# SandeepaInduwaraSamaranayake/SwinVox

Hardware: AMD Instinct MI355X
Metric: views/sec fwd+bwd SwinVox-T 224^2, 32^3 voxel, n_views=8 (higher is better)
Workload: dtype bf16; 1 GPU; SwinVox-T full pipeline (ResNet50[:layer3] || Swin multi-stage, cross-view attention, decoder, merger, refiner), fwd+2xBCE+bwd, train mode, B=64 samples x V=8 views of 224x224 per GPU; global_batch=64, n_views=8, images_per_gpu=512, parallelism=single GPU, launch=eager (one host launch per kernel, three streams)

## Files before the change

include/swinvox_hip.h:

```cpp
#ifndef SWINVOX_HIP_H
#define SWINVOX_HIP_H
#include <stddef.h>
#include <stdint.h>

#ifdef __cplusplus
extern "C" {
#endif

#define SV_OK 0
#define SV_ERR_INVALID (-1)
#define SV_ERR_LAUNCH (-2)

enum { SV_ACT_NONE = 0, SV_ACT_RELU = 1, SV_ACT_GELU = 2, SV_ACT_LRELU = 3 };
#define SV_BN_SLOTS 16
enum { SV_MATH_F32 = 0, SV_MATH_BF16 = 1, SV_MATH_FP8 = 2, SV_MATH_FP8_FULL = 3 };
enum { SV_F32 = 0, SV_BF16 = 1 };

const char* sv_last_error(void);
int sv_version(void);

typedef struct sv_geom {
  int N;
  int Di, Hi, Wi;
  int Do, Ho, Wo;
// ... 14 lines not shown
  double* stats;
  int act;
  float slope;
  const void* act_grad_src;
  int act_grad_kind;
  int ldc;
  int col_off;
} sv_epilogue;

int sv_conv_gather(const void* in, const void* w_packed, void* out, const sv_geom* g, const sv_epilogue* e,
                   int math, int act_dtype, void* stream);
int sv_set_conv_halo(int mode);
int sv_conv_halo_mode(void);
int sv_set_conv_halo_wgrad(int mode);
long long sv_conv_halo_launches(void);
enum { SV_PATH_GATHER = 0,
       SV_PATH_DENSE = 1,
       SV_PATH_WIDE = 2,
       SV_PATH_WIDE_GENERAL = 3,
       SV_PATH_HALO0 = 4, SV_PATH_HALO1 = 5, SV_PATH_HALO2 = 6,
       SV_PATH_HALO_BLOCKED_8X32 = 7, SV_PATH_HALO_BLOCKED_16X16 = 8,
       SV_PATH_WGRAD_TILED = 9,
       SV_PATH_WGRAD_WIDE = 10, SV_PATH_WGRAD_WIDE_SWAP = 11,
       SV_PATH_WGRAD_HALO = 12 };
enum { SV_OPERANDS_F32 = 0, SV_OPERANDS_BF16_F32 = 1, SV_OPERANDS_BF16 = 2 };
typedef struct sv_launch_plan {
  int path;
  int tile_rows, tile_cols;
  int operands;
  int vec;
  int grid_x, grid_y, block;
} sv_launch_plan;
int sv_conv_gather_plan(const void* in, const void* w, void* out, const sv_geom* g, const sv_epilogue* e, int math, int act_dtype, int transposed,
                        sv_launch_plan* plan);
int sv_conv_gather_is_wide(const void* in, const void* w, void* out, const sv_geom* g, const sv_epilogue* e, int math, int act_dtype);
int sv_tconv_gather(const void* in, const void* w_packed, void* out, const sv_geom* g, const sv_epilogue* e,
                    int math, int act_dtype, void* stream);
int sv_conv_wgrad_plan(const void* anchor, int lda, const void* gathered, const sv_geom* g, int cg_valid, int math, int act_dtype,
                       sv_launch_plan* plan);
int sv_conv_wgrad_is_wide(const void* anchor, int lda, const void* gathered, const sv_geom* g, int cg_valid, int math, int act_dtype);
size_t sv_conv_wgrad_workspace_floats(const sv_geom* g);
int sv_conv_wgrad(const void* anchor, int lda, const void* gathered, float* dw, const sv_geom* g, int cg_valid,
                  float* workspace, float* dbias , int math, int act_dtype,
                  void* stream);
int sv_quant_rows_e4m3(const void* src, int src_dtype, int rows, int K, int ld, void* dst_q, int Kp, float* scales, void* stream);
int sv_linear_fp8(const void* xq, const float* sx, const void* wq, const float* sw, void* out, int M, int K, int N, const sv_epilogue* e,
                  int act_dtype, void* stream);
// ... 233 lines not shown
```

swinvox_amd/csrc/igemm.hip:

```cpp
#include "common.h"
#include "conv_halo.h"
#include <stdlib.h>
#include <atomic>
#include <mutex>

namespace sv {

constexpr int PAD_F32 = 4;
#ifndef SV_PAD_BF16
#define SV_PAD_BF16 8
#endif
constexpr int PAD_BF16 = SV_PAD_BF16;

struct Geom {
  int N, Di, Hi, Wi, Do, Ho, Wo, Ci, Co, kd, kh, kw, sd, sh, sw, pd, ph, pw, ldi;
};
struct Epi {
  const float* bias; const void* residual; int ldr; const float* row_scale; int rows_per_scale;
  void* pre_act; double* stats; int act; float slope; const void* act_grad_src; int act_grad_kind; int ldc; int col_off;
};
struct ClassInfo {
  int o0[3];
  int cnt[3];
  int ib0[3];
// ... 545 lines not shown
    for (int mt = 0; mt < MT; ++mt)
#pragma unroll
      for (int nt = 0; nt < NT; ++nt) acc[mt][nt] = (f32x4){0.f, 0.f, 0.f, 0.f};
    for (int kt = 0; kt < nk; ++kt) {
      const int cur = kt & 1;
      if (kt + 1 < nk) load_slab(row0, col0, (kt + 1) * BK);
      mma_slab<true, MT, NT>(As + cur * STAGE, Bs + cur * STAGE, wm * MT * 16, wn * NT * 16, lane, acc);
      if (kt + 1 < nk) store_slab(cur ^ 1);
      __syncthreads();
    }
    int row0n = 0, col0n = 0;
    const bool more = tile_of(++it, row0n, col0n);
    if (more) load_slab(row0n, col0n, 0);
#ifdef SV_IG_PROBE_NOEPI
    if (acc[0][0][0] == 12345.678f) static_cast<AT*>(p.y)[0] = (AT)acc[0][0][1];
#else
    tile_epilogue<true, false, TL, AT>(p, ci, g.Do, g.Ho, g.Wo, Cs, red, acc, row0, col0, Mrows);
    __syncthreads();
#endif
    have = more; row0 = row0n; col0 = col0n;
  }
}

constexpr int GW_BN = 128, GW_BK = 64;
constexpr unsigned GW_NODRAW = 0xFFFFFFFFu;
typedef __attribute__((address_space(1))) const void* gw_gptr_t;
typedef __attribute__((address_space(3))) void* gw_lptr_t;

template <bool GENERAL, int WM, int NPROD, int NST>
__global__ __launch_bounds__((2 * WM + NPROD) * 64, 3) void gemm_wide_kernel(const IGemmArgs p, int ntiles, int* __restrict__ ctr) {
  constexpr int GW_NCONS = 2 * WM, GW_BM = 64 * WM, GW_A_BYTES = GW_BM * GW_BK * 2, GW_STAGE_BYTES = (GW_BM + GW_BN) * GW_BK * 2, GW_STAGES = NST;
  constexpr int PA = GW_BM / 8 / NPROD, PB = GW_BN / 8 / NPROD, LEAD = NST - 1;
  static_assert(PA % 2 == 0 && PB % 2 == 0 && (NST == 2 || NST == 3), "piece parity / ring depth");
  __shared__ __attribute__((aligned(1024))) char smem[GW_STAGES * GW_STAGE_BYTES + 64 + GW_NCONS * 1024];
  const __bf16* __restrict__ X = static_cast<const __bf16*>(p.x);
  const __bf16* __restrict__ Wt = static_cast<const __bf16*>(p.w);
  __bf16* __restrict__ Y = static_cast<__bf16*>(p.y);
  const Geom& g = p.g;
  const Epi& e = p.e;
  const int tid = threadIdx.x, lane = tid & 63, wave = tid >> 6;
  const int Mrows = g.N * g.Do * g.Ho * g.Wo, K = g.Ci, nk = K / GW_BK;
  const int tiles_n = (g.Co + GW_BN - 1) / GW_BN;
  const int xcd = blockIdx.x & 7, cq = ntiles >> 3, cr = ntiles & 7;
  const int cbase = xcd * cq + (xcd < cr ? xcd : cr), csize = cq + (xcd < cr ? 1 : 0);
  typedef __attribute__((address_space(3))) int lds_int;
  lds_int* mbox = (lds_int*)(smem + GW_STAGES * GW_STAGE_BYTES);
// ... 595 lines not shown
  if (g.Hi != g.Ho || g.Wi != g.Wo || g.ldi != g.Ci) return HaloPlan{};
  if (e.bias || e.residual || e.row_scale || e.pre_act || e.act != SV_ACT_NONE || e.act_grad_src || e.ldc != g.Co || e.col_off != 0) return HaloPlan{};
  if (dgrad && e.stats) return HaloPlan{};
  const bool k3 = g.kh == 3 && g.kw == 3 && g.ph == 1 && g.pw == 1, k4 = g.kh == 4 && g.kw == 4 && g.ph == 2 && g.pw == 2;
  if (dgrad && k4 && g.Ci == 64 && g.Co == 16) return conv_halo_plan(2, g.N, g.Hi, g.Wi);
  if (g.Co & 63) return HaloPlan{};
  if (k3) return g.Ci == 64 && g.Co == 64 ? conv_halo_plan(0, g.N, g.Hi, g.Wi) : conv_halo_blocked_plan(g.N, g.Hi, g.Wi, g.Ci, g.Co);
  if (!dgrad && k4 && g.Ci == 16 && g.Co == 64) return conv_halo_plan(1, g.N, g.Hi, g.Wi);
  return HaloPlan{};
}

static bool gemm_wide_ok(const IGemmArgs& a, long long M) {
  static const int enabled = [] { const char* v = getenv("SV_GEMM_WIDE"); return v ? atoi(v) : 1; }();
  const Epi& e = a.e;
  const int K = a.g.Ci, Co = a.g.Co;
  if (!enabled || K % GW_BK || K < 3 * GW_BK || Co < 128 || a.Ktot % 8) return false;
  if (enabled == 1 && e.stats && K < 1024) return false;
  if (enabled == 1 && e.act_grad_src && K < 384) return false;
  if (!rows_16_byte_aligned(a) || ((uintptr_t)a.w & 15)) return false;
  if ((e.stats && (e.residual || e.act_grad_src)) || (e.residual && e.act_grad_src)) return false;
  return (long long)cdiv(M, 256) * cdiv(Co, GW_BN) >= 256;
}

static GatherPlan plan_gather(const IGemmArgs& a, long long M, int ncls, int math, int act, bool tconv, bool counters) {
  const Geom& g = a.g;
  const int Co = g.Co;
  GatherPlan p{};
  const bool v8 = act == SV_BF16 && (g.Ci % 8) == 0 && (g.ldi % 8) == 0 && ((uintptr_t)a.x & 15) == 0;
  p.q.operands = math != SV_MATH_BF16 ? SV_OPERANDS_F32 : act != SV_BF16 ? SV_OPERANDS_BF16_F32 : SV_OPERANDS_BF16;
  p.q.vec = v8 ? 8 : 4;
  p.q.grid_y = 1;
  if (counters && (p.halo = plan_halo(a, math, act, tconv)).kind >= 0) {
    p.q.path = p.halo.kind < 3 ? SV_PATH_HALO0 + p.halo.kind : p.halo.th == 16 ? SV_PATH_HALO_BLOCKED_16X16 : SV_PATH_HALO_BLOCKED_8X32;
    p.q.tile_rows = p.halo.th; p.q.tile_cols = p.halo.tw; p.q.grid_x = p.halo.grid; p.q.block = 256;
    p.counters = true;
    return p;
  }
  const bool dense = !tconv && v8 && g.kd * g.kh * g.kw == 1 && g.sd == 1 && g.sh == 1 && g.sw == 1 &&
                     g.pd == 0 && g.ph == 0 && g.pw == 0 && g.Di == g.Do && g.Hi == g.Ho && g.Wi == g.Wo;
  if (dense && counters && gemm_wide_ok(a, M)) {
    p.q.path = a.e.residual || a.e.act_grad_src ? SV_PATH_WIDE_GENERAL : SV_PATH_WIDE;
    p.q.tile_rows = 256; p.q.tile_cols = GW_BN; p.q.grid_x = 256; p.q.block = 768;
    p.ntiles = cdiv(M, 256) * cdiv(Co, GW_BN);
    p.counters = true;
    return p;
  }
  bool use96 = false;
  if (Co % 96 == 0 && !a.e.stats) {
    auto est = [&](int bm, int bn) {
      const long long tn = cdiv(Co, bn), tiles = (long long)cdiv(M, bm) * tn * ncls;
      return (double)((tiles + 255) / 256) * bm * bn * (1.0 + 0.02 * (tn - 1));
    };
    const double e96 = est(128, 96), e64 = est(128, 64), e128 = Co > 64 ? est(128, 128) : 1e300;
    use96 = e96 <= e64 && e96 <= e128;
  }
  p.tile = Co <= 16 ? TILE_NARROW : use96 ? TILE_96 : Co > 64 && (long long)cdiv(M, 128) * cdiv(Co, 128) * ncls >= 384 ? TILE_BIG : TILE_DEFAULT;
  with_tile(p.tile, [&](auto tl) {
    typedef decltype(tl) TL;
    const int ntiles = cdiv(M, TL::BM) * cdiv(Co, TL::BN), resident = 256 * (TL::NTHR >= 512 ? 2 : 4);
    p.q.tile_rows = TL::BM; p.q.tile_cols = TL::BN; p.q.block = TL::NTHR;
    if (dense && Co > 16) { p.q.path = SV_PATH_DENSE; p.ntiles = ntiles; p.q.grid_x = resident < ntiles ? resident : ntiles; }
    else { p.q.path = SV_PATH_GATHER; p.q.grid_x = ntiles; p.q.grid_y = ncls; }
  });
  return p;
}

template <bool TCONV>
static void launch_gather(const GatherPlan& p, const IGemmArgs& a, int* ctr, hipStream_t s) {
  const dim3 grid(p.q.grid_x, p.q.grid_y), block(p.q.block);
  switch (p.q.path) {
    case SV_PATH_HALO0: case SV_PATH_HALO1: case SV_PATH_HALO2:
      conv_halo_launch(HaloConvArgs{a.x, a.w, a.y, a.e.stats, a.g.N, a.g.Hi, a.g.Wi, TCONV ? 1 : 0}, p.halo, ctr, s);
      return;
    case SV_PATH_HALO_BLOCKED_8X32: case SV_PATH_HALO_BLOCKED_16X16:
      conv_halo_blocked_launch(a.x, a.w, a.y, a.e.stats, a.g.N, a.g.Hi, a.g.Wi, a.g.Ci, a.g.Co, TCONV ? 1 : 0, p.halo, ctr, s);
      return;
    case SV_PATH_WIDE: hipLaunchKernelGGL((gemm_wide_kernel<false, 4, 4, 3>), grid, block, 0, s, a, p.ntiles, ctr); return;
    case SV_PATH_WIDE_GENERAL: hipLaunchKernelGGL((gemm_wide_kernel<true, 4, 4, 3>), grid, block, 0, s, a, p.ntiles, ctr); return;
    default: break;
  }
  with_tile(p.tile, [&](auto tl) {
    typedef decltype(tl) TL;
    if constexpr (!TCONV && TL::BN > 16) {
      if (p.q.path == SV_PATH_DENSE) { hipLaunchKernelGGL((gemm_dense_kernel<TL, __bf16, __bf16, 8>), grid, block, 0, s, a, p.ntiles); return; }
    }
    if (p.q.operands == SV_OPERANDS_F32) hipLaunchKernelGGL((igemm_kernel<false, TCONV, TL, float, float, 4>), grid, block, 0, s, a);
    else if (p.q.operands == SV_OPERANDS_BF16_F32) hipLaunchKernelGGL((igemm_kernel<true, TCONV, TL, float, float, 4>), grid, block, 0, s, a);
    else if (p.q.vec == 8) hipLaunchKernelGGL((igemm_kernel<true, TCONV, TL, __bf16, __bf16, 8>), grid, block, 0, s, a);
    else hipLaunchKernelGGL((igemm_kernel<true, TCONV, TL, __bf16, __bf16, 4>), grid, block, 0, s, a);
  });
}

static int gather_entry(const void* in, const void* w, void* out, const sv_geom* g, const sv_epilogue* e, int math, int act_dtype, bool transposed,
                        hipStream_t s, sv_launch_plan* query) {
  if (int rc = check_common(g, e, in, w, out, act_dtype)) return rc;
  SV_REQUIRE_ACT(act_dtype);
  SV_REQUIRE(act_dtype == SV_F32 || math == SV_MATH_BF16, "igemm: bf16 activations require SV_MATH_BF16");
  IGemmArgs a{};
  a.x = in; a.w = w; a.y = out; a.g = to_geom(g); a.e = to_epi(e);
  a.Ktot = g->kd * g->kh * g->kw * g->Ci;
  long long M = (long long)g->N * g->Do * g->Ho * g->Wo;
// ... 8 lines not shown
          const int r[3] = {rd, rh, rw};
          ClassInfo c{};
          long long m = g->N;
          for (int ax = 0; ax < 3; ++ax) {
            c.r[ax] = r[ax];
            c.T[ax] = r[ax] < Kx[ax] ? (Kx[ax] - r[ax] + S[ax] - 1) / S[ax] : 0;
            int o0 = ((r[ax] - P[ax]) % S[ax] + S[ax]) % S[ax];
            c.o0[ax] = o0;
            c.cnt[ax] = o0 < O[ax] ? (O[ax] - o0 + S[ax] - 1) / S[ax] : 0;
            c.ib0[ax] = (o0 + P[ax] - r[ax]) / S[ax];
            m *= c.cnt[ax];
          }
          if (m > M) M = m;
          a.cls[ncls++] = c;
        }
  }
  GatherPlan p = plan_gather(a, M, ncls, math, act_dtype, transposed, true);
  if (query) { *query = p.q; return SV_OK; }
  if (M == 0) return SV_OK;
  int* ctr = p.counters ? gemm_wide_counters() : nullptr;
  if (p.counters && !ctr) p = plan_gather(a, M, ncls, math, act_dtype, transposed, false);
  if (transposed) launch_gather<true>(p, a, ctr, s);
  else launch_gather<false>(p, a, ctr, s);
  if (p.q.path >= SV_PATH_HALO0) return check_launch(transposed ? "sv_tconv_gather (halo tiles)" : "sv_conv_gather (halo tiles)");
  return check_launch(transposed ? "sv_tconv_gather" : "sv_conv_gather");
}

struct WGradWideArgs {
  const __bf16* P; int ldp; int pcols; const __bf16* Q; int ldq; int qcols;
  float* dw; int ld_dw;
  float* dbias;
  int nslices, ntiles, tiles_p, groups;
};

constexpr int GW_NCONS = 8, GW_NPROD = 4, GW_NTHR = (GW_NCONS + GW_NPROD) * 64, GW_STAGES = 3;
constexpr int GW_A_BYTES = 256 * GW_BK * 2, GW_STAGE_BYTES = (256 + GW_BN) * GW_BK * 2;
template <bool SWAP>
__global__ __launch_bounds__(GW_NTHR, 3) void wgrad_wide_kernel(const WGradWideArgs p) {
  __shared__ __attribute__((aligned(1024))) char smem[GW_STAGES * GW_STAGE_BYTES];
  const int tid = threadIdx.x, lane = tid & 63, wave = tid >> 6;
  const int bl = xcd_remap(blockIdx.x, gridDim.x);
  const int tile = bl % p.ntiles, grp = bl / p.ntiles;
  const int p0 = (tile % p.tiles_p) * 256, q0 = (tile / p.tiles_p) * 128;
  const int sbase = p.nslices / p.groups, srem = p.nslices % p.groups;
  const int s0 = grp * sbase + (grp < srem ? grp : srem), nsl = sbase + (grp < srem ? 1 : 0);
  if (nsl <= 0) return;

// ... 244 lines not shown
    int blocks = cdiv(total, 256); if (blocks > 2048) blocks = 2048;
    hipLaunchKernelGGL(wgrad_unpack_kernel, dim3(blocks), dim3(256), 0, s, workspace, dw, g->Co, g->Ci, cg_valid, taps);
  }
  return check_launch(p.q.path == SV_PATH_WGRAD_HALO ? "sv_conv_wgrad (halo tiles)" : "sv_conv_wgrad");
}

}

using namespace sv;

extern "C" int sv_conv_gather(const void* in, const void* w, void* out, const sv_geom* g, const sv_epilogue* e,
                              int math, int act_dtype, void* stream) {
  return gather_entry(in, w, out, g, e, math, act_dtype, false, (hipStream_t)stream, nullptr);
}
extern "C" int sv_tconv_gather(const void* in, const void* w, void* out, const sv_geom* g, const sv_epilogue* e,
                               int math, int act_dtype, void* stream) {
  return gather_entry(in, w, out, g, e, math, act_dtype, true, (hipStream_t)stream, nullptr);
}
extern "C" int sv_conv_gather_plan(const void* in, const void* w, void* out, const sv_geom* g, const sv_epilogue* e, int math, int act_dtype,
                                   int transposed, sv_launch_plan* plan) {
  SV_REQUIRE(plan, "conv_gather_plan: null plan");
  return gather_entry(in, w, out, g, e, math, act_dtype, transposed != 0, nullptr, plan);
}
extern "C" int sv_conv_gather_is_wide(const void* in, const void* w, void* out, const sv_geom* g, const sv_epilogue* e, int math, int act_dtype) {
  sv_launch_plan q;
  return sv_conv_gather_plan(in, w, out, g, e, math, act_dtype, 0, &q) == SV_OK && (q.path == SV_PATH_WIDE || q.path == SV_PATH_WIDE_GENERAL);
}

extern "C" size_t sv_conv_wgrad_workspace_floats(const sv_geom* g) {
  const int taps = g->kd * g->kh * g->kw;
  return taps == 1 ? 0 : (size_t)g->Co * taps * g->Ci;
}
extern "C" int sv_conv_wgrad(const void* anchor, int lda, const void* gathered, float* dw, const sv_geom* g, int cg_valid,
                             float* workspace, float* dbias, int math, int act_dtype, void* stream) {
  return wgrad_entry(anchor, lda, gathered, dw, g, cg_valid, workspace, dbias, math, act_dtype, (hipStream_t)stream, nullptr);
}
extern "C" int sv_conv_wgrad_plan(const void* anchor, int lda, const void* gathered, const sv_geom* g, int cg_valid, int math, int act_dtype,
                                  sv_launch_plan* plan) {
  SV_REQUIRE(plan, "conv_wgrad_plan: null plan");
  return wgrad_entry(anchor, lda, gathered, nullptr, g, cg_valid, nullptr, nullptr, math, act_dtype, nullptr, plan);
}
extern "C" int sv_conv_wgrad_is_wide(const void* anchor, int lda, const void* gathered, const sv_geom* g, int cg_valid, int math, int act_dtype) {
  sv_launch_plan q;
  return sv_conv_wgrad_plan(anchor, lda, gathered, g, cg_valid, math, act_dtype, &q) == SV_OK &&
         (q.path == SV_PATH_WGRAD_WIDE || q.path == SV_PATH_WGRAD_WIDE_SWAP);
}
// ... 41 lines not shown
```

swinvox_amd/csrc/stencil.hip:

```cpp
#include "common.h"
#include <map>
#include <mutex>
#include <type_traits>

namespace sv {

constexpr int TZ = 4, TY = 8, TX = 8;
constexpr int HZ = TZ + 2, HY = TY + 2, HX = TX + 2;
constexpr int HPOS = HZ * HY * HX;
constexpr int NVOX = TZ * TY * TX;
typedef __attribute__((address_space(3))) bf16x4 lds_bf16x4_t;

__device__ __forceinline__ bf16x4 to_bf16x4(float4 v) {
  bf16x4 b;
  b[0] = (__bf16)v.x; b[1] = (__bf16)v.y; b[2] = (__bf16)v.z; b[3] = (__bf16)v.w;
  return b;
}
__device__ __forceinline__ bf16x4 to_bf16x4(bf16x4 v) { return v; }

__device__ __forceinline__ int xcd_first_tile() {
  const int n = gridDim.x, b = blockIdx.x;
  return (n & 7) == 0 ? (b & 7) * (n >> 3) + (b >> 3) : b;
}

// ... 571 lines not shown
        const int tap = dz * 9 + p0 + pi;
#pragma unroll
        for (int gg = 0; gg < G; ++gg) {
          const f32x4 o = hand[((pi * 3 + dz) * G + gg) * 64];
          const int cm = gg * 16 + lr;
          const int grp = cm / p.c_stride, within = cm - grp * p.c_stride;
          const int ci = grp * p.c_valid + within;
          if (within < p.c_valid && ci < p.cin) {
#pragma unroll
            for (int j = 0; j < 4; ++j) {
              const int co = lg * 4 + j;
              if (co < p.cout) atomicAdd(dst + ((size_t)co * p.cin + ci) * 27 + tap, acc[pi][dz][gg][j] + o[j]);
            }
          }
        }
      }
    }
  }
}

struct TConv4Args {
  const __bf16* x; const __bf16* w;
  const float* bias; __bf16* out; double* stats; int cout; int I, D, H, W, nbricks;
};
constexpr int T4_JZ = 4, T4_JY = 4, T4_JX = 8, T4_HZ = 6, T4_HY = 6, T4_HX = 10, T4_HPOS = T4_HZ * T4_HY * T4_HX;

__global__ __launch_bounds__(256, 2) void tconv4s2_fwd_kernel(const TConv4Args p) {
  __shared__ __attribute__((aligned(16))) __bf16 Xs[T4_HPOS * 32];
  __shared__ __attribute__((aligned(16))) __bf16 Ws[8 * 8 * 256];
  __shared__ __attribute__((aligned(16))) __bf16 Os[8 * 8 * 16 * 8];
  __shared__ float red[4][16];
  const int tid = threadIdx.x, lane = tid & 63, wave = tid >> 6;
  const int lr = lane & 15, lg = lane >> 4;
  for (int i = tid; i < 8 * 8 * 256 / 8; i += 256) {
    const int c8 = (i & 3) * 8, t = (i >> 2) & 7, co = (i >> 5) & 7, cls = i >> 8;
    const int az = cls >> 2, ay = (cls >> 1) & 1, ax = cls & 1, dz = t >> 2, dy = (t >> 1) & 1, dx = t & 1;
    const int kz = az ? 2 - 2 * dz : 3 - 2 * dz, ky = ay ? 2 - 2 * dy : 3 - 2 * dy, kx = ax ? 2 - 2 * dx : 3 - 2 * dx;
    bf16x8 v = VecN<__bf16, 8>::zero();
    if (co < p.cout) v = *reinterpret_cast<const bf16x8*>(p.w + ((size_t)co * 64 + (kz * 4 + ky) * 4 + kx) * 32 + c8);
    *reinterpret_cast<bf16x8*>(Ws + ((cls * 8 + co) * 256) + t * 32 + c8) = v;
  }
  float bias4[4];
#pragma unroll
  for (int j = 0; j < 4; ++j) bias4[j] = (p.bias && lg < 2 && lg * 4 + j < p.cout) ? p.bias[lg * 4 + j] : 0.f;
  double st1[8], st2[8];
#pragma unroll
// ... 26 lines not shown
        if (lr < 8) b[tt] = *reinterpret_cast<const bf16x8*>(Ws + (cls * 8 + lr) * 256 + tt * 32 + lg * 8);
      }
#pragma unroll 2
      for (int g = 0; g < 8; ++g) {
        const int jz = g >> 1, jy = (g & 1) * 2 + yy;
        const int base = ((jz + az) * T4_HY + (jy + ay)) * T4_HX + (xx + ax);
        f32x4 acc = (f32x4){0.f, 0.f, 0.f, 0.f};
#pragma unroll
        for (int tt = 0; tt < 8; ++tt) {
          const int off = ((tt >> 2) * T4_HY + ((tt >> 1) & 1)) * T4_HX + (tt & 1);
          const bf16x8 a = *reinterpret_cast<const bf16x8*>(Xs + (base + off) * 32 + lg * 8);
          acc = __builtin_amdgcn_mfma_f32_16x16x32_bf16(b[tt], a, acc, 0, 0, 0);
        }
        if (lg < 2) {
          bf16x4 o;
#pragma unroll
          for (int j = 0; j < 4; ++j) o[j] = (__bf16)(acc[j] + bias4[j]);
          const int oz = 2 * jz + az, oy = 2 * jy + ay, ox = 2 * xx + ax;
          *reinterpret_cast<bf16x4*>(Os + ((oz * 8 + oy) * 16 + ox) * 8 + lg * 4) = o;
        }
      }
    }
    __syncthreads();
#pragma unroll
    for (int k = 0; k < 4; ++k) {
      const int v = tid + 256 * k;
      const int ox = v & 15, oy = (v >> 4) & 7, oz = v >> 7;
      const bf16x8 o = *reinterpret_cast<const bf16x8*>(Os + v * 8);
      const size_t pos = (((size_t)img * (2 * p.D) + 2 * z0 + oz) * (2 * p.H) + 2 * y0 + oy) * (2 * p.W) + 2 * x0 + ox;
      *reinterpret_cast<bf16x8*>(p.out + pos * 8) = o;
      if (p.stats) {
#pragma unroll
        for (int c = 0; c < 8; ++c) { const double f = (double)(float)o[c]; st1[c] += f; st2[c] += f * f; }
      }
    }
    __syncthreads();
  }
  if (p.stats) {
#pragma unroll
    for (int c = 0; c < 8; ++c) {
      float a = (float)st1[c], b2 = (float)st2[c];
      a = wave_sum(a); b2 = wave_sum(b2);
      if (lane == 0) { red[wave][c] = a; red[wave][8 + c] = b2; }
    }
    __syncthreads();
    if (tid < 16 && (tid & 7) < p.cout) {
      const float v = red[0][tid] + red[1][tid] + red[2][tid] + red[3][tid];
      double* st = p.stats + (size_t)(blockIdx.x % SV_BN_SLOTS) * 2 * p.cout;
      atomicAdd(st + (tid >> 3) * p.cout + (tid & 7), (double)v);
    }
  }
}

}

using namespace sv;

static int resident_per_cu(const void* kernel, int threads = 256) {
  static std::mutex mu;
  static std::map<const void*, int> cache;
  std::lock_guard<std::mutex> lk(mu);
  auto it = cache.find(kernel);
  if (it != cache.end()) return it->second;
  int n = 0;
  if (hipOccupancyMaxActiveBlocksPerMultiprocessor(&n, kernel, threads, 0) != hipSuccess || n < 1) { (void)hipGetLastError(); n = 1; }
  cache[kernel] = n;
  return n;
}

static int stencil_check(int I, int D, int H, int W) {
  SV_REQUIRE(I > 0 && D % 8 == 0 && H % TY == 0 && W % TX == 0, "stencil3: grid %dx%dx%d must be a multiple of the 8x8x8 brick", D, H, W);
  return SV_OK;
}

#define SV_STENCIL_LAUNCH(GG, NTT, VV)                                                                                     \
  do {                                                                                                                    \
    constexpr int nthr = StencilBrickF<GG>::NTHR;                                                                         \
    const int nt_ = I * (D / StencilBrickF<GG>::TZV) * (H / TY) * (W / TX);                                               \
    a.ntiles = nt_;                                                                                                       \
// ... 56 lines not shown
  const bool sweep = sweep_env ? atoi(sweep_env) != 0 : true;
  SV_DISPATCH_ACT(act_dtype,
    const void* k1 = sweep ? (const void*)stencil3_wgrad_sweep_kernel<1, AT> : (const void*)stencil3_wgrad_kernel<1, AT>;
    const void* k3 = sweep ? (const void*)stencil3_wgrad_sweep_kernel<3, AT> : (const void*)stencil3_wgrad_kernel<3, AT>;
    const int per_cu = groups == 1 ? resident_per_cu(k1, StencilBrick<1>::NTHR) : resident_per_cu(k3, StencilBrick<3>::NTHR);
    const int resident = 256 * per_cu;
    const int blocks = ntiles < resident ? ntiles : resident;
    StencilWArgsT<AT> a{static_cast<const AT*>(x), ldx, cin_load, x_plane_stride, static_cast<const AT*>(dy), lddy, cout_load, dw, workspace, dbias, cout, cin, c_stride, c_valid,
                        I, D, H, W, ntiles};
    if (groups == 1 && sweep) hipLaunchKernelGGL((stencil3_wgrad_sweep_kernel<1, AT>), dim3(blocks), dim3(StencilBrick<1>::NTHR), 0, s, a);
    else if (groups == 1) hipLaunchKernelGGL((stencil3_wgrad_kernel<1, AT>), dim3(blocks), dim3(StencilBrick<1>::NTHR), 0, s, a);
    else if (sweep) hipLaunchKernelGGL((stencil3_wgrad_sweep_kernel<3, AT>), dim3(blocks), dim3(StencilBrick<3>::NTHR), 0, s, a);
    else hipLaunchKernelGGL((stencil3_wgrad_kernel<3, AT>), dim3(blocks), dim3(StencilBrick<3>::NTHR), 0, s, a););
  if (workspace) hipLaunchKernelGGL(stencil_wgrad_fold_kernel, dim3(cdiv(cout * cin * 27, 256)), dim3(256), 0, s, workspace, dw, cout * cin * 27);
  return check_launch("sv_stencil3_wgrad");
}

extern "C" int sv_tconv4s2_fwd(const void* x, const void* w_packed, const float* bias, void* out, double* stats, int I, int D, int H, int W,
                               int cin, int cout, void* stream) {
  SV_REQUIRE(x && w_packed && out && I > 0, "tconv4s2_fwd: null argument");
  SV_REQUIRE(cin == 32 && cout > 0 && cout <= 8, "tconv4s2_fwd: built for 32 input and <= 8 output channels (got %d -> %d)", cin, cout);
  SV_REQUIRE(D % T4_JZ == 0 && H % T4_JY == 0 && W % T4_JX == 0, "tconv4s2_fwd: input grid %dx%dx%d must be a multiple of the 4x4x8 brick", D, H, W);
  SV_REQUIRE((((uintptr_t)x | (uintptr_t)w_packed | (uintptr_t)out) & 15) == 0, "tconv4s2_fwd: operands must be 16-byte aligned");
  TConv4Args a{static_cast<const __bf16*>(x), static_cast<const __bf16*>(w_packed), bias, static_cast<__bf16*>(out), stats, cout, I, D, H, W,
               I * (D / T4_JZ) * (H / T4_JY) * (W / T4_JX)};
  const int blocks = a.nbricks < 512 ? a.nbricks : 512;
  hipLaunchKernelGGL(tconv4s2_fwd_kernel, dim3(blocks), dim3(256), 0, (hipStream_t)stream, a);
  return check_launch("sv_tconv4s2_fwd");
}
```

swinvox_amd/hip.py:

```python
from __future__ import annotations

import ctypes as C
import os
import threading

import torch

_HERE = os.path.dirname(os.path.abspath(__file__))
LIB_PATH = os.environ.get("SV_HIP_LIB") or os.path.join(_HERE, "libswinvox_hip.so")

ACT_NONE, ACT_RELU, ACT_GELU, ACT_LRELU = 0, 1, 2, 3
MATH_F32, MATH_BF16, MATH_FP8, MATH_FP8_FULL = 0, 1, 2, 3
F32, BF16 = 0, 1


class Geom(C.Structure):
    _fields_ = [(n, C.c_int) for n in ("N", "Di", "Hi", "Wi", "Do", "Ho", "Wo", "Ci", "Co", "kd", "kh", "kw",
                                        "sd", "sh", "sw", "pd", "ph", "pw", "ldi")]


class Epilogue(C.Structure):
    _fields_ = [("bias", C.c_void_p), ("residual", C.c_void_p), ("ldr", C.c_int), ("row_scale", C.c_void_p),
                ("rows_per_scale", C.c_int), ("pre_act", C.c_void_p), ("stats", C.c_void_p), ("act", C.c_int),
                ("slope", C.c_float), ("act_grad_src", C.c_void_p), ("act_grad_kind", C.c_int), ("ldc", C.c_int),
                ("col_off", C.c_int)]


class LaunchPlan(C.Structure):
    _fields_ = [(n, C.c_int) for n in ("path", "tile_rows", "tile_cols", "operands", "vec", "grid_x", "grid_y", "block")]


(PATH_GATHER, PATH_DENSE, PATH_WIDE, PATH_WIDE_GENERAL, PATH_HALO0, PATH_HALO1, PATH_HALO2, PATH_HALO_BLOCKED_8X32, PATH_HALO_BLOCKED_16X16,
 PATH_WGRAD_TILED, PATH_WGRAD_WIDE, PATH_WGRAD_WIDE_SWAP, PATH_WGRAD_HALO) = range(13)
OPERANDS_F32, OPERANDS_BF16_F32, OPERANDS_BF16 = 0, 1, 2


class PackDesc(C.Structure):
    _fields_ = [("src", C.c_void_p), ("dst", C.c_void_p), ("A", C.c_int), ("B", C.c_int), ("T", C.c_int), ("swap", C.c_int),
                ("rows_out", C.c_int), ("inner_out", C.c_int), ("block0", C.c_int), ("reserved", C.c_int)]


class AugSample(C.Structure):
    _fields_ = [("bg", C.c_float * 3), ("jitter_value", C.c_float * 3), ("jitter_order", C.c_int * 3), ("noise", C.c_float * 3),
                ("perm", C.c_int * 3), ("mean", C.c_float * 3), ("std", C.c_float * 3)]


_P, _I, _L, _F, _U, _D = C.c_void_p, C.c_int, C.c_longlong, C.c_float, C.c_uint32, C.c_double
_ACT_TYPED = {
    "sv_conv_gather", "sv_tconv_gather", "sv_conv_wgrad", "sv_stencil3_fwd", "sv_stencil3_wgrad", "sv_colsum",
    "sv_layernorm_fwd", "sv_layernorm_quant_fwd", "sv_layernorm_quant_mx_fwd", "sv_layernorm_bwd", "sv_ln_image_fwd", "sv_ln_image_bwd", "sv_bn_stats", "sv_scale_shift_act", "sv_bn_bwd", "sv_scale_shift_act_signs", "sv_bn_bwd_signs", "sv_scale_shift_act2_signs", "sv_bn_bwd2_signs",
    "sv_window_attention_fwd", "sv_window_attention_fwd_mxq", "sv_window_attention_bwd", "sv_cross_view_attention_fwd", "sv_cross_view_attention_bwd",
    "sv_transpose", "sv_add_n", "sv_axpby", "sv_relu_bwd", "sv_maxpool2d_fwd", "sv_maxpool2d_bwd", "sv_avgpool2_fwd", "sv_avgpool2_bwd",
    "sv_decoder_seed_fwd", "sv_decoder_seed_bwd", "sv_maxpool3d_fwd", "sv_maxpool3d_bwd", "sv_dropout", "sv_rowscale",
    "sv_dwconv2x2_fwd", "sv_dwconv2x2_bwd", "sv_upsample3to7_add_fwd", "sv_upsample3to7_bwd",
    "sv_cva_downsample_fwd", "sv_cva_downsample_bwd", "sv_cva_upsample_add_fwd", "sv_cva_upsample_bwd", "sv_decoder_head_fwd", "sv_decoder_head_bwd",
    "sv_merge_views_fwd", "sv_merge_views_bwd", "sv_stem_space_to_depth", "sv_encoder_prep", "sv_encoder_prep_bwd", "sv_bn_act_maxpool_fwd", "sv_bn_maxpool_bwd", "sv_bn_act_maxpool3d_fwd", "sv_bn_maxpool3d_bwd", "sv_head_pack_x", "sv_head_unpack_dx", "sv_swin_attn_block_fwd", "sv_swin_attn_block_fwd_mx", "sv_swin_attn_block_bwd",
# ... 55 lines not shown
    "sv_bn_stats": (_I, [_P, _L, _I, _I, _P]),
    "sv_bn_finalize": (_I, [_P, _L, _P, _P, _P, _P, _F, _F, _I, _P, _P, _P, _P, _I]),
    "sv_scale_shift_act": (_I, [_P, _I, _P, _P, _P, _I, _P, _I, _L, _I, _I, _F]),
    "sv_bn_bwd": (_I, [_P, _I, _P, _I, _P, _I, _P, _P, _P, _L, _I, _I, _F, _I, _P, _I, _P, _I, _P, _P, _P, _P, _P]),
    "sv_bn_signs_supported": (_I, None, [_I]),
    "sv_scale_shift_act_signs": (_I, [_P, _I, _P, _P, _P, _I, _P, _I, _L, _I, _I, _F, _P]),
    "sv_bn_bwd_signs": (_I, [_P, _I, _P, _P, _I, _P, _P, _P, _L, _I, _I, _F, _I, _P, _I, _P, _I, _P, _P, _P]),
    "sv_scale_shift_act2_signs": (_I, [_P, _I, _P, _P, _P, _I, _P, _P, _P, _I, _L, _I, _P]),
    "sv_bn_bwd2_signs": (_I, [_P, _I, _P, _P, _I, _P, _P, _P, _P, _I, _P, _P, _P, _L, _I, _P, _I, _P, _I, _P, _P, _P, _P, _P, _P]),
    "sv_window_attention_fwd": (_I, [_P, _P, _P, _I, _I, _I, _I, _I, _I, _I]),
    "sv_window_attention_fwd_mxq": (_I, [_P, _P, _P, _I, _I, _I, _I, _I, _I, _I, _P, _I, _P]),
    "sv_window_attention_bwd_workspace_floats": (C.c_size_t, None, [_I]),
    "sv_window_attention_windows_per_group": (_I, None, [_I, _I, _I, _I, _I, _I]),
    "sv_window_attention_bwd": (_I, [_P, _P, _P, _P, _P, _P, _I, _I, _I, _I, _I, _I, _I]),
    "sv_stem_space_to_depth": (_I, [_P, _P, _I]),
    "sv_bn_act_maxpool_fwd": (_I, [_P, _P, _P, _P, _P, _I, _I, _I, _I, _I, _F]),
    "sv_bn_maxpool_bwd": (_I, [_P, _P, _P, _P, _P, _P, _P, _P, _I, _I, _I, _I, _I, _F, _I, _P, _P, _P, _P]),
    "sv_bn_act_maxpool3d_fwd": (_I, [_P, _P, _P, _P, _P, _I, _I, _I, _I, _I, _I, _F]),
    "sv_bn_maxpool3d_bwd": (_I, [_P, _P, _P, _P, _P, _P, _P, _P, _I, _I, _I, _I, _I, _I, _F, _I, _P, _P, _P, _P]),
    "sv_set_conv_halo": (_I, None, [_I]),
    "sv_conv_halo_mode": (_I, None),
    "sv_set_conv_halo_wgrad": (_I, None, [_I]),
    "sv_conv_halo_launches": (_L, None),
    "sv_encoder_prep": (_I, [_P, _I, _P, _P, _I, _I]),
    "sv_encoder_prep_bwd": (_I, [_P, _P, _P, _I, _I, _I]),
    "sv_head_pack_x": (_I, [_P, _P, _I, _I]),
    "sv_head_unpack_dx": (_I, [_P, _P, _I, _I]),
    "sv_stem_pack": (_I, [_P, _P, _I]),
    "sv_stem_unpack_grad": (_I, [_P, _P]),
    "sv_stem_native": (_I, [_P, _P]),
    "sv_merger_pack": (_I, [_P, _P, _I, _I, _I, _I]),
    "sv_swin_mlp_supported": (_I, None, [_I]),
    "sv_swin_mlp_pack": (_I, [_P, _P, _P, _I]),
    "sv_swin_mlp_fwd": (_I, [_P, _P, _P, _P, _P, _P, _P, _P, _I, _L, _I, _F]),
    "sv_swin_mlp_bwd": (_I, [_P, _P, _P, _P, _P, _P, _P, _P, _I, _P, _P, _L, _I, _F]),
    "sv_swin_mlp_wgrad": (_I, [_P, _P, _P, _P, _P, _P, _P, _P, _I, _P, _P, _P, _P, _L, _I, _F]),
    "sv_swin_mlp_mx_supported": (_I, None, [_I]),
    "sv_swin_mlp_mx_pack_bytes": (_L, None, [_I]),
    "sv_swin_mlp_mx_pack": (_I, [_P, _P, _P, _P, _P, _I]),
    "sv_swin_mlp_fwd_mx": (_I, [_P, _P, _P, _P, _P, _P, _P, _P, _I, _L, _I, _F]),
    "sv_swin_mlp_mx_launches": (_L, None),
    "sv_swin_mlp_bwd_mx_supported": (_I, None, [_I]),
    "sv_swin_mlp_bwd_mx_pack_bytes": (_L, None, [_I]),
    "sv_swin_mlp_bwd_mx_pack": (_I, [_P, _P, _P, _P, _P, _P, _P, _I]),
    "sv_swin_mlp_bwd_mx": (_I, [_P, _P, _P, _P, _P, _P, _P, _P, _I, _P, _P, _L, _I, _F]),
    "sv_swin_mlp_bwd_mx_launches": (_L, None),
# ... 191 lines not shown
```

Before: 4999 views/s.

## Route tiny-M dense GEMMs and 4x4x4 stride-2 tconv fwd/dgrad to specialized kernels

```diff
diff --git a/include/swinvox_hip.h b/include/swinvox_hip.h
--- a/include/swinvox_hip.h
+++ b/include/swinvox_hip.h
@@ -60,7 +60,11 @@
        SV_PATH_HALO_BLOCKED_8X32 = 7, SV_PATH_HALO_BLOCKED_16X16 = 8,
        SV_PATH_WGRAD_TILED = 9,
        SV_PATH_WGRAD_WIDE = 10, SV_PATH_WGRAD_WIDE_SWAP = 11,
-       SV_PATH_WGRAD_HALO = 12 };
+       SV_PATH_WGRAD_HALO = 12,
+       SV_PATH_SKINNY = 13,
+       SV_PATH_TCONV_BRICK = 14,
+       SV_PATH_TCONV_BRICK_DGRAD = 15 };
+int sv_set_tail_kernels(int mask);
 enum { SV_OPERANDS_F32 = 0, SV_OPERANDS_BF16_F32 = 1, SV_OPERANDS_BF16 = 2 };
 typedef struct sv_launch_plan {
   int path;
diff --git a/swinvox_amd/csrc/igemm.hip b/swinvox_amd/csrc/igemm.hip
--- a/swinvox_amd/csrc/igemm.hip
+++ b/swinvox_amd/csrc/igemm.hip
@@ -1,5 +1,6 @@
 #include "common.h"
 #include "conv_halo.h"
+#include "stencil.h"
 #include <stdlib.h>
 #include <atomic>
 #include <mutex>
@@ -591,6 +592,103 @@
   }
 }
 
+constexpr int SK_NW = 8, SK_NS = 4, SK_BN = 16, SK_BK = 64;
+template <int MB> struct SkinnyStage { bf16x8 w[2]; bf16x8 x[MB][2]; };
+
+template <int MB>
+__global__ __launch_bounds__(SK_NW * 64, 2) void gemm_skinny_kernel(const IGemmArgs p) {
+  __shared__ __attribute__((aligned(16))) float part[SK_NW][MB][64][4];
+  const Geom& g = p.g;
+  const Epi& e = p.e;
+  const int tid = threadIdx.x, lane = tid & 63, wave = tid >> 6, lr = lane & 15, lg = lane >> 4;
+  const int M = g.N * g.Do * g.Ho * g.Wo, nch = g.Ci / SK_BK;
+  const int n0 = blockIdx.x * SK_BN;
+  const __bf16* __restrict__ wrow = static_cast<const __bf16*>(p.w) + (size_t)(n0 + lr) * p.Ktot + lg * 8;
+  const __bf16* __restrict__ xrow[MB];
+  bool xok[MB];
+#pragma unroll
+  for (int mb = 0; mb < MB; ++mb) {
+    const int m = mb * 16 + lr;
+    xok[mb] = m < M;
+    xrow[mb] = static_cast<const __bf16*>(p.x) + (size_t)(xok[mb] ? m : 0) * g.ldi + lg * 8;
+  }
+  SkinnyStage<MB> st[SK_NS];
+  auto load = [&](SkinnyStage<MB>& s, int i) {
+    const int c = wave + SK_NW * i;
+    if (c < nch) {
+      const int k0 = c * SK_BK;
+#pragma unroll
+      for (int ks = 0; ks < 2; ++ks) s.w[ks] = VecN<__bf16, 8>::load(wrow + k0 + ks * 32);
+#pragma unroll
+      for (int mb = 0; mb < MB; ++mb)
+#pragma unroll
+        for (int ks = 0; ks < 2; ++ks) s.x[mb][ks] = xok[mb] ? VecN<__bf16, 8>::load(xrow[mb] + k0 + ks * 32) : VecN<__bf16, 8>::zero();
+    } else {
+#pragma unroll
+      for (int ks = 0; ks < 2; ++ks) {
+        s.w[ks] = VecN<__bf16, 8>::zero();
+#pragma unroll
+        for (int mb = 0; mb < MB; ++mb) s.x[mb][ks] = VecN<__bf16, 8>::zero();
+      }
+    }
+  };
+  f32x4 acc[MB];
+#pragma unroll
+  for (int mb = 0; mb < MB; ++mb) acc[mb] = (f32x4){0.f, 0.f, 0.f, 0.f};
+#pragma unroll
+  for (int s = 0; s < SK_NS; ++s) load(st[s], s);
+  const int nmine = wave < nch ? (nch - wave + SK_NW - 1) / SK_NW : 0;
+  for (int i0 = 0; i0 < nmine; i0 += SK_NS) {
+#pragma unroll
+    for (int s = 0; s < SK_NS; ++s) {
+#pragma unroll
+      for (int ks = 0; ks < 2; ++ks)
+#pragma unroll
+        for (int mb = 0; mb < MB; ++mb)
+          acc[mb] = __builtin_amdgcn_mfma_f32_16x16x32_bf16(st[s].w[ks], st[s].x[mb][ks], acc[mb], 0, 0, 0);
+      load(st[s], i0 + s + SK_NS);
+    }
+  }
+#pragma unroll
+  for (int mb = 0; mb < MB; ++mb) *reinterpret_cast<f32x4*>(&part[wave][mb][lane][0]) = acc[mb];
+  __syncthreads();
+  const int m = wave * 16 + lr;
+  if (wave >= MB || m >= M) return;
+  f32x4 sum = *reinterpret_cast<const f32x4*>(&part[0][wave][lane][0]);
+#pragma unroll
+  for (int w = 1; w < SK_NW; ++w) sum += *reinterpret_cast<const f32x4*>(&part[w][wave][lane][0]);
+  const int n = n0 + lg * 4;
+  const size_t o = (size_t)m * e.ldc + e.col_off + n;
+  float v[4];
+#pragma unroll
+  for (int j = 0; j < 4; ++j) v[j] = sum[j] + (e.bias ? e.bias[n + j] : 0.f);
+  if (e.act_grad_src) {
+    float a[4];
+    ldnf<4>(static_cast<const __bf16*>(e.act_grad_src) + o, a);
+    if (e.act_grad_kind == SV_ACT_GELU) {
+#pragma unroll
+      for (int j = 0; j < 4; j += 2) {
+        const f32x2 dg = gelu_grad_fast2((f32x2){a[j], a[j + 1]});
+        v[j] *= dg[0]; v[j + 1] *= dg[1];
+      }
+    } else {
+#pragma unroll
+      for (int j = 0; j < 4; ++j) v[j] *= act_grad_t<true>(a[j], e.act_grad_kind, e.slope);
+    }
+  }
+  if (e.act == SV_ACT_GELU) {
+#pragma unroll
+    for (int j = 0; j < 4; j += 2) {
+      const f32x2 gl = gelu_fast2((f32x2){v[j], v[j + 1]});
+      v[j] = gl[0]; v[j + 1] = gl[1];
+    }
+  } else {
+#pragma unroll
+    for (int j = 0; j < 4; ++j) v[j] = apply_act_t<true>(v[j], e.act, e.slope);
+  }
+  stnf<4>(static_cast<__bf16*>(p.y) + o, v);
+}
+
 constexpr int GW_BN = 128, GW_BK = 64;
 constexpr unsigned GW_NODRAW = 0xFFFFFFFFu;
 typedef __attribute__((address_space(1))) const void* gw_gptr_t;
@@ -1232,6 +1330,41 @@
   return (long long)cdiv(M, 256) * cdiv(Co, GW_BN) >= 256;
 }
 
+static std::atomic<int>& tail_mask() {
+  static std::atomic<int> m{[] { const char* v = getenv("SV_TAIL_KERNELS"); return v ? atoi(v) & 15 : 7; }()};
+  return m;
+}
+constexpr long long SK_MIN_KCO = 1LL << 16;
+static bool skinny_ok(const IGemmArgs& a, long long M) {
+  const int mask = tail_mask().load(std::memory_order_relaxed);
+  const Epi& e = a.e;
+  if (!(mask & 1) || M < 1 || M > 64 || a.g.Ci < SK_BK || a.g.Ci % SK_BK || a.g.Co % SK_BN) return false;
+  if (e.residual || e.row_scale || e.pre_act || e.stats) return false;
+  if (!rows_16_byte_aligned(a) || (((uintptr_t)a.w | (uintptr_t)a.x) & 15) || a.Ktot % 8) return false;
+  return (mask & 8) != 0 || (long long)a.g.Ci * a.g.Co >= SK_MIN_KCO;
+}
+static bool tconv_brick_ok(const IGemmArgs& a, int math, int act) {
+  const Geom& g = a.g;
+  const Epi& e = a.e;
+  if (!(tail_mask().load(std::memory_order_relaxed) & 4) || math != SV_MATH_BF16 || act != SV_BF16) return false;
+  if (g.kd != 4 || g.kh != 4 || g.kw != 4 || g.sd != 2 || g.sh != 2 || g.sw != 2 || g.pd != 1 || g.ph != 1 || g.pw != 1) return false;
+  if (g.Do != 2 * g.Di || g.Ho != 2 * g.Hi || g.Wo != 2 * g.Wi || g.Di % 4 || g.Hi % 4 || g.Wi % 8) return false;
+  if (g.Ci != 32 || g.ldi != 32 || g.Co > 8 || e.ldc != g.Co || e.col_off != 0) return false;
+  if (e.residual || e.row_scale || e.pre_act || e.stats || e.act != SV_ACT_NONE || e.act_grad_src) return false;
+  return (((uintptr_t)a.x | (uintptr_t)a.w | (uintptr_t)a.y) & 15) == 0;
+}
+
+static bool tconv_brick_dgrad_ok(const IGemmArgs& a, int math, int act) {
+  const Geom& g = a.g;
+  const Epi& e = a.e;
+  if (!(tail_mask().load(std::memory_order_relaxed) & 2) || math != SV_MATH_BF16 || act != SV_BF16) return false;
+  if (g.kd != 4 || g.kh != 4 || g.kw != 4 || g.sd != 2 || g.sh != 2 || g.sw != 2 || g.pd != 1 || g.ph != 1 || g.pw != 1) return false;
+  if (g.Di != 2 * g.Do || g.Hi != 2 * g.Ho || g.Wi != 2 * g.Wo || g.Do % 4 || g.Ho % 4 || g.Wo % 8) return false;
+  if (g.Ci != 8 || g.ldi != 8 || g.Co != 32 || e.ldc != 32 || e.col_off != 0) return false;
+  if (e.bias || e.residual || e.row_scale || e.pre_act || e.stats || e.act != SV_ACT_NONE || e.act_grad_src) return false;
+  return (((uintptr_t)a.x | (uintptr_t)a.w | (uintptr_t)a.y) & 15) == 0;
+}
+
 static GatherPlan plan_gather(const IGemmArgs& a, long long M, int ncls, int math, int act, bool tconv, bool counters) {
   const Geom& g = a.g;
   const int Co = g.Co;
@@ -1248,6 +1381,20 @@
   }
   const bool dense = !tconv && v8 && g.kd * g.kh * g.kw == 1 && g.sd == 1 && g.sh == 1 && g.sw == 1 &&
                      g.pd == 0 && g.ph == 0 && g.pw == 0 && g.Di == g.Do && g.Hi == g.Ho && g.Wi == g.Wo;
+  if (tconv && tconv_brick_ok(a, math, act)) {
+    const int nbricks = g.N * (g.Di / 4) * (g.Hi / 4) * (g.Wi / 8);
+    p.q.path = SV_PATH_TCONV_BRICK; p.q.tile_rows = 4 * 4 * 8; p.q.tile_cols = 8; p.q.grid_x = nbricks < 512 ? nbricks : 512; p.q.block = 256;
+    return p;
+  }
+  if (!tconv && tconv_brick_dgrad_ok(a, math, act)) {
+    const int nbricks = g.N * (g.Do / 4) * (g.Ho / 4) * (g.Wo / 8);
+    p.q.path = SV_PATH_TCONV_BRICK_DGRAD; p.q.tile_rows = 4 * 4 * 8; p.q.tile_cols = 32; p.q.grid_x = nbricks < 512 ? nbricks : 512; p.q.block = 256;
+    return p;
+  }
+  if (dense && math == SV_MATH_BF16 && skinny_ok(a, M)) {
+    p.q.path = SV_PATH_SKINNY; p.q.tile_rows = 64; p.q.tile_cols = SK_BN; p.q.grid_x = Co / SK_BN; p.q.block = SK_NW * 64;
+    return p;
+  }
   if (dense && counters && gemm_wide_ok(a, M)) {
     p.q.path = a.e.residual || a.e.act_grad_src ? SV_PATH_WIDE_GENERAL : SV_PATH_WIDE;
     p.q.tile_rows = 256; p.q.tile_cols = GW_BN; p.q.grid_x = 256; p.q.block = 768;
@@ -1287,6 +1434,17 @@
       return;
     case SV_PATH_WIDE: hipLaunchKernelGGL((gemm_wide_kernel<false, 4, 4, 3>), grid, block, 0, s, a, p.ntiles, ctr); return;
     case SV_PATH_WIDE_GENERAL: hipLaunchKernelGGL((gemm_wide_kernel<true, 4, 4, 3>), grid, block, 0, s, a, p.ntiles, ctr); return;
+    case SV_PATH_SKINNY: {
+      const int M = a.g.N * a.g.Do * a.g.Ho * a.g.Wo;
+      if (M <= 16) hipLaunchKernelGGL(gemm_skinny_kernel<1>, grid, block, 0, s, a);
+      else if (M <= 32) hipLaunchKernelGGL(gemm_skinny_kernel<2>, grid, block, 0, s, a);
+      else hipLaunchKernelGGL(gemm_skinny_kernel<4>, grid, block, 0, s, a);
+      return;
+    }
+    case SV_PATH_TCONV_BRICK_DGRAD: tconv4s2_dgrad_launch(a.x, a.w, a.y, a.g.N, a.g.Do, a.g.Ho, a.g.Wo, p.q.grid_x, s); return;
+    case SV_PATH_TCONV_BRICK:
+      tconv4s2_fwd_launch(a.x, a.w, a.e.bias, a.y, nullptr, a.g.N, a.g.Di, a.g.Hi, a.g.Wi, a.g.Co, a.e.ldc, p.q.grid_x, s);
+      return;
     default: break;
   }
   with_tile(p.tile, [&](auto tl) {
@@ -1341,7 +1499,7 @@
   if (p.counters && !ctr) p = plan_gather(a, M, ncls, math, act_dtype, transposed, false);
   if (transposed) launch_gather<true>(p, a, ctr, s);
   else launch_gather<false>(p, a, ctr, s);
-  if (p.q.path >= SV_PATH_HALO0) return check_launch(transposed ? "sv_tconv_gather (halo tiles)" : "sv_conv_gather (halo tiles)");
+  if (p.q.path >= SV_PATH_HALO0 && p.q.path <= SV_PATH_HALO_BLOCKED_16X16) return check_launch(transposed ? "sv_tconv_gather (halo tiles)" : "sv_conv_gather (halo tiles)");
   return check_launch(transposed ? "sv_tconv_gather" : "sv_conv_gather");
 }
 
@@ -1632,6 +1790,11 @@
   SV_REQUIRE(plan, "conv_gather_plan: null plan");
   return gather_entry(in, w, out, g, e, math, act_dtype, transposed != 0, nullptr, plan);
 }
+extern "C" int sv_set_tail_kernels(int mask) {
+  SV_REQUIRE(mask >= 0 && mask <= 15, "sv_set_tail_kernels: mask %d (bit 0 skinny dense, bit 1 brick data gradient, bit 2 transposed-convolution brick, bit 3 skinny below its threshold)", mask);
+  sv::tail_mask().store(mask, std::memory_order_relaxed);
+  return SV_OK;
+}
 extern "C" int sv_conv_gather_is_wide(const void* in, const void* w, void* out, const sv_geom* g, const sv_epilogue* e, int math, int act_dtype) {
   sv_launch_plan q;
   return sv_conv_gather_plan(in, w, out, g, e, math, act_dtype, 0, &q) == SV_OK && (q.path == SV_PATH_WIDE || q.path == SV_PATH_WIDE_GENERAL);
diff --git a/swinvox_amd/csrc/stencil.h b/swinvox_amd/csrc/stencil.h
--- /dev/null
+++ b/swinvox_amd/csrc/stencil.h
@@ -0,0 +1,10 @@
+#pragma once
+#include <hip/hip_runtime.h>
+
+namespace sv {
+
+void tconv4s2_fwd_launch(const void* x, const void* w, const float* bias, void* out, double* stats, int I, int D, int H, int W, int cout, int ldc,
+                         int blocks, hipStream_t stream);
+void tconv4s2_dgrad_launch(const void* dy, const void* w, void* dx, int I, int D, int H, int W, int blocks, hipStream_t stream);
+
+}
diff --git a/swinvox_amd/csrc/stencil.hip b/swinvox_amd/csrc/stencil.hip
--- a/swinvox_amd/csrc/stencil.hip
+++ b/swinvox_amd/csrc/stencil.hip
@@ -1,4 +1,5 @@
 #include "common.h"
+#include "stencil.h"
 #include <map>
 #include <mutex>
 #include <type_traits>
@@ -617,6 +618,7 @@
 struct TConv4Args {
   const __bf16* x; const __bf16* w;
   const float* bias; __bf16* out; double* stats; int cout; int I, D, H, W, nbricks;
+  int ldc;
 };
 constexpr int T4_JZ = 4, T4_JY = 4, T4_JX = 8, T4_HZ = 6, T4_HY = 6, T4_HX = 10, T4_HPOS = T4_HZ * T4_HY * T4_HX;
 
@@ -689,6 +691,22 @@
       }
     }
     __syncthreads();
+    if (p.ldc != 8) {
+      const int pieces = 2 * p.cout;
+      for (int q = tid; q < 64 * pieces; q += 256) {
+        const int row = q / pieces, pc = q - row * pieces, oy = row & 7, oz = row >> 3;
+        bf16x8 o;
+#pragma unroll
+        for (int j = 0; j < 8; ++j) {
+          const int el = pc * 8 + j, ox = el / p.cout, c = el - ox * p.cout;
+          o[j] = Os[(row * 16 + ox) * 8 + c];
+        }
+        const size_t pos = (((size_t)img * (2 * p.D) + 2 * z0 + oz) * (2 * p.H) + 2 * y0 + oy) * (2 * p.W) + 2 * x0;
+        *reinterpret_cast<bf16x8*>(p.out + pos * p.cout + pc * 8) = o;
+      }
+      __syncthreads();
+      continue;
+    }
 #pragma unroll
     for (int k = 0; k < 4; ++k) {
       const int v = tid + 256 * k;
@@ -719,9 +737,100 @@
   }
 }
 
+struct TConv4DgradArgs {
+  const __bf16* dy; const __bf16* w;
+  __bf16* dx;
+  int I, D, H, W, nbricks;
+};
+constexpr int T4D_HZ = 10, T4D_HY = 10, T4D_HX = 18, T4D_SLOTS = T4D_HZ * T4D_HY * T4D_HX, T4D_ROW = 12, T4D_PLANE = T4D_HZ * T4D_HY * T4D_ROW;
+constexpr int T4D_PF = (T4D_SLOTS + 255) / 256;
+
+__global__ __launch_bounds__(256, 2) void tconv4s2_dgrad_kernel(const TConv4DgradArgs p) {
+  __shared__ __attribute__((aligned(16))) __bf16 Ys[2 * T4D_PLANE * 8];
+  const int tid = threadIdx.x, lane = tid & 63, wave = tid >> 6;
+  const int lr = lane & 15, lg = lane >> 4;
+  bf16x8 b[16][2];
+#pragma unroll
+  for (int ks = 0; ks < 16; ++ks)
+#pragma unroll
+    for (int ct = 0; ct < 2; ++ct)
+      b[ks][ct] = *reinterpret_cast<const bf16x8*>(p.w + ((size_t)((lr >> 2) * 8 + ct * 4 + (lr & 3)) * 64 + ks * 4 + lg) * 8);
+  const int bz = p.D / T4_JZ, by = p.H / T4_JY, bx = p.W / T4_JX;
+  const int Dy = 2 * p.D, Hy = 2 * p.H, Wy = 2 * p.W;
+  int img, z0, y0, x0;
+  auto decode = [&](int brick) {
+    int t = brick;
+    x0 = (t % bx) * T4_JX; t /= bx;
+    y0 = (t % by) * T4_JY; t /= by;
+    z0 = (t % bz) * T4_JZ; img = t / bz;
+  };
+  bf16x8 pf[T4D_PF];
+  auto fetch = [&](int brick) {
+    int fi, fz, fy, fx;
+    { int t = brick; fx = (t % bx) * T4_JX; t /= bx; fy = (t % by) * T4_JY; t /= by; fz = (t % bz) * T4_JZ; fi = t / bz; }
+#pragma unroll
+    for (int i = 0; i < T4D_PF; ++i) {
+      const int h = tid + 256 * i;
+      const int hx = h % T4D_HX, t2 = h / T4D_HX, hy = t2 % T4D_HY, hz = t2 / T4D_HY;
+      const int z = 2 * fz - 1 + hz, y = 2 * fy - 1 + hy, x = 2 * fx - 1 + hx;
+      pf[i] = VecN<__bf16, 8>::zero();
+      if (h < T4D_SLOTS && (unsigned)z < (unsigned)Dy && (unsigned)y < (unsigned)Hy && (unsigned)x < (unsigned)Wy)
+        pf[i] = *reinterpret_cast<const bf16x8*>(p.dy + ((((size_t)fi * Dy + z) * Hy + y) * Wy + x) * 8);
+    }
+  };
+  int brick = blockIdx.x;
+  if (brick < p.nbricks) fetch(brick);
+  const int yy = lr >> 3, xx = lr & 7;
+  const int lane_slot = (lg & 1) * T4D_PLANE + xx + (lg >> 1);
+  while (brick < p.nbricks) {
+#pragma unroll
+    for (int i = 0; i < T4D_PF; ++i) {
+      const int h = tid + 256 * i;
+      const int hx = h % T4D_HX, row = h / T4D_HX;
+      if (h < T4D_SLOTS) *reinterpret_cast<bf16x8*>(Ys + ((hx & 1) * T4D_PLANE + row * T4D_ROW + (hx >> 1)) * 8) = pf[i];
+    }
+    __syncthreads();
+    decode(brick);
+    const int next = brick + gridDim.x;
+    if (next < p.nbricks) fetch(next);
+#pragma unroll 1
+    for (int g = 0; g < 2; ++g) {
+      const int jy = 2 * g + yy;
+      f32x4 acc[2] = {(f32x4){0.f, 0.f, 0.f, 0.f}, (f32x4){0.f, 0.f, 0.f, 0.f}};
+#pragma unroll
+      for (int ks = 0; ks < 16; ++ks) {
+        const int row = (2 * wave + (ks >> 2)) * T4D_HY + 2 * jy + (ks & 3);
+        const bf16x8 a = *reinterpret_cast<const bf16x8*>(Ys + (row * T4D_ROW + lane_slot) * 8);
+#pragma unroll
+        for (int ct = 0; ct < 2; ++ct) acc[ct] = __builtin_amdgcn_mfma_f32_16x16x32_bf16(b[ks][ct], a, acc[ct], 0, 0, 0);
+      }
+      bf16x8 o;
+#pragma unroll
+      for (int j = 0; j < 4; ++j) { o[j] = (__bf16)acc[0][j]; o[4 + j] = (__bf16)acc[1][j]; }
+      const size_t pos = (((size_t)img * p.D + z0 + wave) * p.H + y0 + jy) * p.W + x0 + xx;
+      *reinterpret_cast<bf16x8*>(p.dx + pos * 32 + lg * 8) = o;
+    }
+    __syncthreads();
+    brick = next;
+  }
+}
+
 }
 
 using namespace sv;
+
+void sv::tconv4s2_dgrad_launch(const void* dy, const void* w, void* dx, int I, int D, int H, int W, int blocks, hipStream_t stream) {
+  TConv4DgradArgs a{static_cast<const __bf16*>(dy), static_cast<const __bf16*>(w), static_cast<__bf16*>(dx), I, D, H, W,
+                    I * (D / T4_JZ) * (H / T4_JY) * (W / T4_JX)};
+  hipLaunchKernelGGL(tconv4s2_dgrad_kernel, dim3(blocks), dim3(256), 0, stream, a);
+}
+
+void sv::tconv4s2_fwd_launch(const void* x, const void* w, const float* bias, void* out, double* stats, int I, int D, int H, int W, int cout, int ldc,
+                             int blocks, hipStream_t stream) {
+  TConv4Args a{static_cast<const __bf16*>(x), static_cast<const __bf16*>(w), bias, static_cast<__bf16*>(out), stats, cout, I, D, H, W,
+               I * (D / T4_JZ) * (H / T4_JY) * (W / T4_JX), ldc};
+  hipLaunchKernelGGL(tconv4s2_fwd_kernel, dim3(blocks), dim3(256), 0, stream, a);
+}
 
 static int resident_per_cu(const void* kernel, int threads = 256) {
   static std::mutex mu;
@@ -824,9 +933,7 @@
   SV_REQUIRE(cin == 32 && cout > 0 && cout <= 8, "tconv4s2_fwd: built for 32 input and <= 8 output channels (got %d -> %d)", cin, cout);
   SV_REQUIRE(D % T4_JZ == 0 && H % T4_JY == 0 && W % T4_JX == 0, "tconv4s2_fwd: input grid %dx%dx%d must be a multiple of the 4x4x8 brick", D, H, W);
   SV_REQUIRE((((uintptr_t)x | (uintptr_t)w_packed | (uintptr_t)out) & 15) == 0, "tconv4s2_fwd: operands must be 16-byte aligned");
-  TConv4Args a{static_cast<const __bf16*>(x), static_cast<const __bf16*>(w_packed), bias, static_cast<__bf16*>(out), stats, cout, I, D, H, W,
-               I * (D / T4_JZ) * (H / T4_JY) * (W / T4_JX)};
-  const int blocks = a.nbricks < 512 ? a.nbricks : 512;
-  hipLaunchKernelGGL(tconv4s2_fwd_kernel, dim3(blocks), dim3(256), 0, (hipStream_t)stream, a);
+  const int nbricks = I * (D / T4_JZ) * (H / T4_JY) * (W / T4_JX);
+  tconv4s2_fwd_launch(x, w_packed, bias, out, stats, I, D, H, W, cout, 8, nbricks < 512 ? nbricks : 512, (hipStream_t)stream);
   return check_launch("sv_tconv4s2_fwd");
 }
diff --git a/swinvox_amd/hip.py b/swinvox_amd/hip.py
--- a/swinvox_amd/hip.py
+++ b/swinvox_amd/hip.py
@@ -31,7 +31,9 @@
 
 
 (PATH_GATHER, PATH_DENSE, PATH_WIDE, PATH_WIDE_GENERAL, PATH_HALO0, PATH_HALO1, PATH_HALO2, PATH_HALO_BLOCKED_8X32, PATH_HALO_BLOCKED_16X16,
- PATH_WGRAD_TILED, PATH_WGRAD_WIDE, PATH_WGRAD_WIDE_SWAP, PATH_WGRAD_HALO) = range(13)
+ PATH_WGRAD_TILED, PATH_WGRAD_WIDE, PATH_WGRAD_WIDE_SWAP, PATH_WGRAD_HALO, PATH_SKINNY, PATH_TCONV_BRICK,
+ PATH_TCONV_BRICK_DGRAD) = range(16)
+TAIL_SKINNY, TAIL_TCONV_BRICK_DGRAD, TAIL_TCONV_BRICK = 1, 2, 4
 OPERANDS_F32, OPERANDS_BF16_F32, OPERANDS_BF16 = 0, 1, 2
 
 
@@ -133,6 +135,7 @@
     "sv_conv_halo_mode": (_I, None),
     "sv_set_conv_halo_wgrad": (_I, None, [_I]),
     "sv_conv_halo_launches": (_L, None),
+    "sv_set_tail_kernels": (_I, None, [_I]),
     "sv_encoder_prep": (_I, [_P, _I, _P, _P, _I, _I]),
     "sv_encoder_prep_bwd": (_I, [_P, _P, _P, _I, _I, _I]),
     "sv_head_pack_x": (_I, [_P, _P, _I, _I]),
```

New measurement: 5047 views/s, median of 6. No clear change (+1.0%).
